# zju3dv/clean-pvnet

Hardware: NVIDIA H100
Metric: ransac_vote_throughput (higher is better)
Workload: dtype f32

## Files before the change

clean_pvnet_b200/csrc/api.cu:

```cuda
#include <cmath>
#include <cstdarg>
#include <cstdio>
#include <cstring>
#include <new>
#include <vector>
#include "kernels.h"

using namespace pvb;

namespace {

thread_local char g_err[512] = "";

int fail(int code, const char *fmt, ...)
{
    va_list ap;
    va_start(ap, fmt);
    vsnprintf(g_err, sizeof(g_err), fmt, ap);
    va_end(ap);
    return code;
}

int cuda_fail(cudaError_t e, const char *what)
{
// ... 12 lines not shown
thread_local std::vector<cudaEvent_t> g_prof_pool;

cudaEvent_t prof_event()
{
    if (!g_prof_pool.empty()) { cudaEvent_t e = g_prof_pool.back(); g_prof_pool.pop_back(); return e; }
    cudaEvent_t e = nullptr;
    cudaEventCreate(&e);
    return e;
}

ProfCall *prof_begin(bool head)
{
    if (g_prof_every <= 0 || (g_prof_tick++ % (unsigned)g_prof_every) != 0) return nullptr;
    ProfCall pc;
    for (auto &e : pc.ev) e = prof_event();
    pc.head = head;
    g_prof_calls.push_back(pc);
    return &g_prof_calls.back();
}

inline void prof_start(ProfCall *pc, int stage, cudaStream_t st) { if (pc && stage == 0) cudaEventRecord(pc->ev[0], st); }
inline void prof_end(ProfCall *pc, int stage, cudaStream_t st) { if (pc) cudaEventRecord(pc->ev[stage + 1], st); }

int default_capacity(const pvb_desc *d)
{
    const long long HW = (long long)d->H * d->W;
    long long cap = d->capacity;
    if (cap <= 0) {
        const long long mn = d->max_num < 0 ? 0 : d->max_num;
        cap = mn + (long long)ceil(8.0 * sqrt((double)mn)) + 64;
    }
    if (cap > HW) cap = HW;
    cap = (cap + 31) / 32 * 32;
    return (int)cap;
}

int check_desc(const pvb_desc *d)
{
    if (!d) return fail(PVB_ERR_INVALID, "descriptor is NULL");
    if (d->B < 0 || d->H <= 0 || d->W <= 0 || d->K <= 0 || d->hn <= 0)
        return fail(PVB_ERR_INVALID, "bad shape B=%d H=%d W=%d K=%d hn=%d", d->B, d->H, d->W, d->K, d->hn);
    if ((long long)d->H * d->W > (1ll << 30)) return fail(PVB_ERR_INVALID, "image too large (H*W > 2^30)");
    if (d->B > 65535 || d->K > 65535) return fail(PVB_ERR_INVALID, "B and K must be <= 65535");
    if ((long long)d->K * ((d->hn + 511) / 512) > 65535) return fail(PVB_ERR_INVALID, "K*ceil(hn/512) must be <= 65535");
    if (d->mask_dtype < PVB_MASK_U8 || d->mask_dtype > PVB_MASK_F64) return fail(PVB_ERR_INVALID, "bad mask_dtype %d", d->mask_dtype);
    if (d->select_mode != PVB_SELECT_BYTE && d->select_mode != PVB_SELECT_EQ1)
        return fail(PVB_ERR_INVALID, "bad select_mode %d", d->select_mode);
    return PVB_OK;
}

int make_layout(const pvb_desc *d, pvb_layout *L)
{
    const int rc = check_desc(d);
    if (rc) return rc;
    const size_t B = (size_t)d->B, K = (size_t)d->K, hn = (size_t)d->hn;
    const int nwords = (int)(((long long)d->H * d->W + 31) / 32);
    const int nblocks = (nwords + 127) / 128;
    const int cap = default_capacity(d);
    const int splits = refit_splits_for(cap);
    size_t off = 0;
    auto take = [&](size_t bytes) { const size_t o = off; off = align_up(off + bytes); return o; };
    L->status = take(4 * sizeof(int));
    L->fgsum = take(B * sizeof(unsigned long long));
    L->nz = take(B * sizeof(int));
    L->tn = take(B * sizeof(int));
    L->state = take(B * sizeof(int));
    L->refit_ticket = take(B * K * sizeof(int));
    L->ticket = take(B * sizeof(int));
    L->blocktot = take(B * nblocks * sizeof(int));
    L->bits = take(B * nwords * sizeof(uint32_t));
    L->xy = take(B * cap * sizeof(float2));
    L->dirs = take(B * K * cap * sizeof(float2));
    L->hyp = take(B * K * hn * sizeof(float2));
    L->counts = take(B * K * hn * sizeof(int));
    L->win = take(B * K * sizeof(float2));
    L->refit_partial = take(B * K * splits * 5 * sizeof(double));
    const size_t ncells = (size_t)((d->H + PRUNE_CELL - 1) / PRUNE_CELL) * ((d->W + PRUNE_CELL - 1) / PRUNE_CELL);
    L->prune_cells = take(B * K * ncells * PRUNE_REC * sizeof(int));
    L->prune_key = take(B * K * hn * sizeof(int));
    L->prune_list = take(2 * B * K * hn * sizeof(int));
    L->prune_len = take(2 * B * K * sizeof(int));
    take(B * K * ncells * 4 * PRUNE_REC * sizeof(int));
    take(B * K * hn * sizeof(int));
    L->total = off;
    L->nwords = nwords;
    L->nblocks = nblocks;
    L->capacity = cap;
    L->refit_splits = splits;
    L->prune_ncells = (int)ncells;
    return PVB_OK;
}

struct Plan {
    pvb_layout L;
    SelectArgs s;
    VoteArgs v;
    float2 *win;
    RefitScratch refit;
    PruneArgs prune;
};

int make_plan(const pvb_desc *d, const void *mask, const float *vertex, const int32_t *idxs,
              const float *selection, void *ws, size_t ws_bytes, uint32_t tag_idx, uint32_t tag_sel, Plan *P)
{
    int rc = make_layout(d, &P->L);
    if (rc) return rc;
    if (!mask || !vertex) return fail(PVB_ERR_INVALID, "mask/vertex is NULL");
    if (!ws || ws_bytes < P->L.total) return fail(PVB_ERR_WORKSPACE, "workspace too small: need %zu bytes, got %zu", P->L.total, ws_bytes);
    if (reinterpret_cast<uintptr_t>(ws) & 255u) return fail(PVB_ERR_WORKSPACE, "workspace must be 256-byte aligned");
    char *w = static_cast<char *>(ws);
    const pvb_layout &L = P->L;
    SelectArgs &s = P->s;
    s.mask = mask; s.mask_dtype = d->mask_dtype; s.select_mode = d->select_mode;
    s.msb = d->mask_stride[0]; s.msy = d->mask_stride[1]; s.msx = d->mask_stride[2];
    s.vertex = vertex;
    for (int i = 0; i < 5; ++i) s.vs[i] = d->vertex_stride[i];
    s.selection = selection;
    s.B = d->B; s.H = d->H; s.W = d->W; s.K = d->K; s.nwords = L.nwords; s.nblocks = L.nblocks; s.cap = L.capacity;
    s.min_num = d->min_num; s.max_num = d->max_num; s.img_base = d->img_base;
    s.seed = d->seed; s.tag_sel = d->rng_tag_sel ? (uint32_t)d->rng_tag_sel : tag_sel;
    s.rowwise_gather = 0;
    s.seg_classes = 0; s.seg_cs = 0; s.mask_out = nullptr;
    s.bits = reinterpret_cast<uint32_t *>(w + L.bits);
    s.blocktot = reinterpret_cast<unsigned *>(w + L.blocktot);
    s.ticket = reinterpret_cast<int *>(w + L.ticket);
    s.fgsum = reinterpret_cast<unsigned long long *>(w + L.fgsum);
    s.nz = reinterpret_cast<int *>(w + L.nz);
    s.tn = reinterpret_cast<int *>(w + L.tn);
    s.state = reinterpret_cast<int *>(w + L.state);
    s.status = reinterpret_cast<int *>(w + L.status);
    s.xy = reinterpret_cast<float2 *>(w + L.xy);
    s.dirs = reinterpret_cast<float2 *>(w + L.dirs);
    VoteArgs &v = P->v;
    v.B = d->B; v.K = d->K; v.hn = d->hn; v.cap = L.capacity; v.W = d->W; v.H = d->H;
    v.thresh = d->inlier_thresh;
    v.tn = s.tn; v.state = s.state; v.xy = s.xy;
    v.dirs = s.dirs; v.idxs = idxs; v.seed = d->seed;
    v.tag_idx = d->rng_tag_idx ? (uint32_t)d->rng_tag_idx : tag_idx;
    v.img_base = d->img_base;
    v.hyp = reinterpret_cast<float2 *>(w + L.hyp);
    v.counts = reinterpret_cast<int *>(w + L.counts);
    P->win = reinterpret_cast<float2 *>(w + L.win);
    P->refit.partial = reinterpret_cast<double *>(w + L.refit_partial);
    P->refit.ticket = reinterpret_cast<int *>(w + L.refit_ticket);
    P->refit.splits = L.refit_splits;
    P->prune.cells = reinterpret_cast<int *>(w + L.prune_cells);
    P->prune.key = reinterpret_cast<int *>(w + L.prune_key);
    P->prune.list = reinterpret_cast<int *>(w + L.prune_list);
    P->prune.len = reinterpret_cast<int *>(w + L.prune_len);
    const size_t BK = (size_t)d->B * d->K;
    const size_t prune_sub = align_up(L.prune_len + 2 * BK * sizeof(int));
    P->prune.sub = reinterpret_cast<int *>(w + prune_sub);
    P->prune.b2 = reinterpret_cast<int *>(w + align_up(prune_sub + BK * L.prune_ncells * 4 * PRUNE_REC * sizeof(int)));
    P->prune.ticket = P->refit.ticket;
    P->prune.ncx = (d->W + PRUNE_CELL - 1) / PRUNE_CELL;
    P->prune.ncells = L.prune_ncells;
    P->prune.cos_w = P->prune.sin_w = 0.f;
    return PVB_OK;
}

cudaError_t run_vote(const Plan &P, bool prune, cudaStream_t st)
{
    PruneArgs q = P.prune;
    if (prune && prune_setup(P.v, q)) return launch_vote_pruned(P.v, q, st);
    return launch_vote(P.v, false, false, st);
}

int run_select(const Plan &P, cudaStream_t st)
{
    cudaError_t e = cudaMemsetAsync(P.s.status, 0, P.L.bits, st);
    if (e != cudaSuccess) return cuda_fail(e, "memset(header)");
    e = launch_select(P.s, st);
    if (e != cudaSuccess) return cuda_fail(e, "select kernels");
    return PVB_OK;
}

int run_front(const Plan &P, bool prune, cudaStream_t st, ProfCall *pc)
{
    prof_start(pc, PVB_STAGE_SELECT, st);
    int rc = run_select(P, st);
    if (rc) return rc;
    prof_end(pc, PVB_STAGE_SELECT, st);
    prof_start(pc, PVB_STAGE_GENERATE, st);
    cudaError_t e = launch_generate(P.v, true, st);
    if (e != cudaSuccess) return cuda_fail(e, "generate kernel");
    prof_end(pc, PVB_STAGE_GENERATE, st);
    prof_start(pc, PVB_STAGE_VOTE, st);
    e = run_vote(P, prune, st);
    if (e != cudaSuccess) return cuda_fail(e, "vote kernel");
    prof_end(pc, PVB_STAGE_VOTE, st);
    return PVB_OK;
}

}

struct pvb_exchange {
    int rank, world, slots, device;
    size_t bytes_per_rank;
    size_t status_off, total;
    char *local;
    char *peer[PVB_MAX_PEERS];
    bool ipc_opened[PVB_MAX_PEERS];
    bool connected;
};

namespace {

int exchange_push_args(pvb_exchange *ex, uint64_t seq, size_t nbytes, PeerPush *pp)
{
    memset(pp, 0, sizeof(*pp));
    if (!ex) return PVB_OK;
    if (!ex->connected) return fail(PVB_ERR_INVALID, "exchange is not connected (pvb_exchange_connect*)");
    if (seq == 0 || (uint32_t)seq == 0) return fail(PVB_ERR_INVALID, "seq must be >= 1 and not a multiple of 2^32");
    if (nbytes > ex->bytes_per_rank) return fail(PVB_ERR_INVALID, "result block (%zu bytes) exceeds the exchange's bytes_per_rank (%zu)", nbytes, ex->bytes_per_rank);
    const size_t slot = (size_t)((seq - 1) % (uint64_t)ex->slots);
    const size_t words = ex->bytes_per_rank / sizeof(float);
    pp->world = ex->world;
    pp->seq = (uint32_t)seq;
    for (int r = 0; r < ex->world; ++r)
        pp->recv[r] = reinterpret_cast<uint2 *>(ex->peer[r]) + (slot * ex->world + ex->rank) * words;
    return PVB_OK;
}

size_t mask_elt_bytes(int dt)
{
    switch (dt) {
    case PVB_MASK_U8: case PVB_MASK_I8: return 1;
    case PVB_MASK_I16: return 2;
    case PVB_MASK_I32: case PVB_MASK_F32: return 4;
    default: return 8;
    }
}

}

extern "C" {
// ... 918 lines not shown
```

clean_pvnet_b200/csrc/kernels.h:

```cpp
#pragma once
#include <cuda_runtime.h>
#include <stdint.h>
#include "../../include/pvnet_vote_b200.h"
#include "pnp_core.cuh"

namespace pvb {

struct SelectArgs {
    const void *mask;
    int mask_dtype, select_mode;
    long long msb, msy, msx;
    const float *vertex;
    long long vs[5];
    const float *selection;
    int B, H, W, K, nwords, nblocks, cap, min_num, max_num, img_base;
    int rowwise_gather;
    int seg_classes;
    long long seg_cs;
    long long *mask_out;
    uint64_t seed;
    uint32_t tag_sel;
    uint32_t *bits;
    unsigned *blocktot;
    int *ticket;
    unsigned long long *fgsum;
    int *nz, *tn, *state, *status;
    float2 *xy, *dirs;
};
cudaError_t launch_select(const SelectArgs &a, cudaStream_t st);

struct VoteArgs {
    int B, K, hn, cap, W, H;
    float thresh;
    const int *tn;
    const int *state;
    const float2 *xy;
    const float2 *dirs;
    const int32_t *idxs;
    uint64_t seed;
    uint32_t tag_idx;
    int img_base;
    float2 *hyp;
    int *counts;
};
cudaError_t launch_generate(const VoteArgs &a, bool chained, cudaStream_t st);
cudaError_t launch_vote(const VoteArgs &a, bool zero_counts, bool chained, cudaStream_t st);

constexpr int PRUNE_CELL = 32;
constexpr int PRUNE_SUB = PRUNE_CELL / 2;
constexpr int PRUNE_NBIN = 128;
constexpr int PRUNE_REC = 4 + PRUNE_NBIN / 2;
constexpr int PRUNE_M = 128;
constexpr int PRUNE_MAX_HN = 2048;
constexpr int PRUNE_MIN_UNITS = 32;
static_assert(PRUNE_CELL * PRUNE_CELL < 65536, "a cell's prefix counts fit 16 bits");
struct PruneArgs {
    int *cells;
    int *sub;
    int *key;
    int *b2;
    int *list;
    int *len;
    int *ticket;
    int ncx, ncells;
    float cos_w, sin_w;
};
bool prune_setup(const VoteArgs &a, PruneArgs &q);
cudaError_t launch_vote_pruned(const VoteArgs &a, const PruneArgs &q, cudaStream_t st);
cudaError_t launch_vote_list(const VoteArgs &a, const int *list, const int *len, int max_len, cudaStream_t st);
cudaError_t launch_vote_list_slices(const VoteArgs &a, const int *list, const int *len, int max_len, cudaStream_t st);
void set_vote_tuning(int variant);
void set_gather_tuning(int mode);
struct RefitScratch { double *partial; int *ticket; int splits; };
int refit_splits_for(int cap);
constexpr int PVB_MAX_PEERS = 16;
struct PeerPush {
    int world;
    unsigned int seq;
    uint2 *recv[PVB_MAX_PEERS];
};
cudaError_t launch_refit(const VoteArgs &a, float2 *win, const RefitScratch &rs, float *out_kpt, const PeerPush &pp,
                         cudaStream_t st);
struct ExchangeCounts { int n[PVB_MAX_PEERS]; };
cudaError_t launch_exchange_wait(const uint2 *recv, unsigned int seq, float *out, int world, int stride_words,
                                 const ExchangeCounts &counts, unsigned long long timeout_ns, int *status, cudaStream_t st);
cudaError_t launch_covariance(const VoteArgs &a, const float *mean, float *out_cov, const PeerPush &pp, cudaStream_t st);

cudaError_t launch_pnp_weights(const float *cov, float *w, int n, cudaStream_t st);

constexpr int PNP_FUSED_MAX_PN = 64;
struct PnpArgs {
    const double *pts2d;
    const double *wgt2d;
    const float *kpt2d;
    const float *cov;
    const float *weights;
    float *weights_out;
    const double *pts3d;
    const double *K;
    const double *init_rt;
    double *init_out;
    double *result_rt;
    int *info;
    double *pose;
    int n, pn;
    long long pts3d_stride, k_stride;
    PnpOptions opt;
};
cudaError_t launch_pnp_batch(const PnpArgs &a, cudaStream_t st);
cudaError_t launch_pnp_iterative(const PnpArgs &a, cudaStream_t st);

struct NnPlan { int qchunks, nsplit, slice; };
NnPlan nn_plan(int b, int pn1, int pn2);
size_t nn_workspace_bytes(int b, int pn1, int pn2);
size_t add_metric_workspace_bytes(int n, int pn, int syn, size_t *partial_offset);
cudaError_t launch_nearest_point(const float *ref, const float *que, int *idxs, int b, int pn1, int pn2, int dim,
                                 bool exclude_self, void *workspace, cudaStream_t st);
cudaError_t launch_add_metric(const double *model, const double *pose_pred, const double *pose_gt, double *mean_dist, int n,
                              int pn, bool syn, void *workspace, cudaStream_t st);
size_t pose_metrics_workspace_bytes(int n, int pn);
cudaError_t launch_pose_metrics(const double *model, const double *pose_pred, const double *pose_gt, const double *K,
                                long long k_stride, double *proj2d, double *trans_cm, double *angle_deg, int n, int pn,
                                void *workspace, cudaStream_t st);
cudaError_t launch_mask_iou(const void *pred, int pred_dtype, const long long *ps, const void *gt, int gt_dtype,
                            const long long *gs, long long *inter, long long *uni, int B, int H, int W, cudaStream_t st);

size_t render_workspace_bytes(int n, int F);
cudaError_t launch_render_depth(const float *pts, int V, const int *faces, int F, const double *poses, int n,
                                const double *K, long long k_stride, float *depth, int H, int W, double znear,
                                double zfar, void *workspace, cudaStream_t st);
struct VsdArgs {
    const float *depth_test, *depth_est, *depth_gt;
    const int *pairs;
    const double *K;
    long long k_stride;
    int n, B, n_est, n_gt, est_base, gt_base, H, W;
    double delta, tau;
    double *e;
};
size_t vsd_workspace_bytes(int n);
cudaError_t launch_vsd(const VsdArgs &a, void *workspace, cudaStream_t st);

struct VoteLossArgs {
    const float *pred;
    long long ps[4];
    const void *mask;
    int mask_dtype;
    long long msb, msy, msx;
    const double *kpt;
    int B, H, W, K;
    float *out;
    double *partial;
    long long *wpart;
// ... 19 lines not shown
```

clean_pvnet_b200/csrc/prune.cu:

```cuda
#include <cmath>
#include <math_constants.h>
#include "common.cuh"
#include "kernels.h"

namespace pvb {

template <bool EXACT = false>
__device__ __forceinline__ float pseudo_angle(float x, float y)
{
    const bool xn = x < 0.f, yn = y < 0.f;
    const float num = (xn == yn) ? fabsf(y) : fabsf(x), den = fabsf(x) + fabsf(y);
    const float off = yn ? (xn ? 2.f : 3.f) : (xn ? 1.f : 0.f);
    return off + (EXACT ? __fdiv_rn(num, den) : __fdividef(num, den));
}

__device__ int first_row_at(const float2 *xy, int n, float y)
{
    const int lane = threadIdx.x & 31;
    int lo = 0, hi = n;
    while (hi > lo) {
        const int step = (hi - lo + 31) / 32;
        const int p = lo + lane * step;
        const unsigned below = __ballot_sync(0xffffffffu, p < hi && __ldg(&xy[p].y) < y);
        const int nb = __popc(below);
// ... 214 lines not shown
            __syncthreads();
        }
    }
}

__device__ void plan_pass1(const VoteArgs &a, const PruneArgs &q, size_t bk, int *s_key, int *s_cnt, int *s_w, int *s_sel)
{
    const int tid = threadIdx.x, lane = tid & 31, warp = tid >> 5;
    const int hn = a.hn, M = min(PRUNE_M, hn);
    int *key = q.key + bk * hn;
    int top = 0;
    for (int h = tid; h < hn; h += BOUND_THREADS) {
        const int v = __ldcg(key + h);
        s_key[h] = v;
        top = max(top, v);
    }
    top = __reduce_max_sync(0xffffffffu, top);
    if (lane == 0) s_w[warp] = top;
    __syncthreads();
    for (int w = 0; w < BOUND_WARPS; ++w) top = max(top, s_w[w]);
    int thr = 0, need = M;
    for (int hi = 32 - __clz(top | 1); hi > 0;) {
        const int lo = max(0, hi - 8);
        for (int i = tid; i < 256; i += BOUND_THREADS) s_cnt[i] = 0;
        __syncthreads();
        for (int h = tid; h < hn; h += BOUND_THREADS) {
            const int v = s_key[h];
            if ((v >> hi) == (thr >> hi)) atomicAdd(&s_cnt[(v >> lo) & ((1 << (hi - lo)) - 1)], 1);
        }
        __syncthreads();
        if (warp == 0) {
            int c[8], own = 0;
#pragma unroll
            for (int e = 0; e < 8; ++e) { c[e] = s_cnt[8 * lane + e]; own += c[e]; }
            int suf = own;
#pragma unroll
            for (int o = 1; o < 32; o <<= 1) {
                const int t = __shfl_down_sync(0xffffffffu, suf, o);
                if (lane + o < 32) suf += t;
            }
            const unsigned ok = __ballot_sync(0xffffffffu, suf >= need);
            if (lane == 31 - __clz(ok)) {
                int above = suf - own;
#pragma unroll
                for (int e = 7; e >= 0; --e) {
                    if (above + c[e] >= need) { s_sel[0] = 8 * lane + e; s_sel[1] = need - above; break; }
                    above += c[e];
                }
            }
        }
        __syncthreads();
        thr |= s_sel[0] << lo;
        need = s_sel[1];
        hi = lo;
    }
    const int per = (hn + 32 * BOUND_WARPS - 1) / (32 * BOUND_WARPS) * 32;
    const int h0 = warp * per, h1 = min(hn, h0 + per);
    int gt = 0, eq = 0;
    for (int h = h0 + lane; h - lane < h1; h += 32) {
        const int v = h < h1 ? s_key[h] : -1;
        gt += __popc(__ballot_sync(0xffffffffu, v > thr));
        eq += __popc(__ballot_sync(0xffffffffu, v == thr));
    }
    int *s_gt = s_w, *s_eq = s_w + BOUND_WARPS;
    __syncthreads();
    if (lane == 0) { s_gt[warp] = gt; s_eq[warp] = eq; }
    __syncthreads();
    gt = eq = 0;
    for (int w = 0; w < warp; ++w) { gt += s_gt[w]; eq += s_eq[w]; }
    int *list = q.list + bk * hn;
    const unsigned below = (1u << lane) - 1u;
    for (int h = h0 + lane; h - lane < h1; h += 32) {
        const int v = h < h1 ? s_key[h] : -1;
        const unsigned mg = __ballot_sync(0xffffffffu, v > thr), me = __ballot_sync(0xffffffffu, v == thr);
        const int g = gt + __popc(mg & below), e = eq + __popc(me & below);
        if (v > thr || (v == thr && e < need)) {
            list[g + min(e, need)] = h;
            key[h] = -1;
        }
        gt += __popc(mg);
        eq += __popc(me);
    }
    if (tid == 0) q.len[bk] = M;
}

__global__ void __launch_bounds__(BOUND_THREADS, 2048 / BOUND_THREADS)
prune_bound_kernel(VoteArgs a, PruneArgs q)
{
    const int tid = threadIdx.x;
    const int part = tid / BOUND_HYPS, hl = tid % BOUND_HYPS;
    const int h = blockIdx.x * BOUND_HYPS + hl, k = blockIdx.y, b = blockIdx.z;
    const size_t bk = (size_t)b * a.K + k;
    const int tn = max(0, min(a.tn[b], a.cap));
    __shared__ __align__(16) int s_rec[2][STAGE_RECS * PRUNE_REC];
    __shared__ int s_idx[3 * BOUND_THREADS];
    __shared__ int s_part[BOUND_SPLIT][BOUND_HYPS];
    __shared__ int s_w[2 * BOUND_WARPS];
    __shared__ int s_sel[2];
    const float2 hp = (h < a.hn) ? a.hyp[bk * a.hn + h] : make_float2(0.f, 0.f);
    grid_dep_wait();
    grid_dep_launch_dependents();
    int bound = 0;
    stream_records<BOUND_THREADS>(q.cells + bk * q.ncells * PRUNE_REC, PRUNE_REC, q.ncells, &s_rec[0][0], s_idx, s_w,
                                  [&](const int *rec, int n) {
        const int r0 = part * n / BOUND_SPLIT, r1 = (part + 1) * n / BOUND_SPLIT;
        count_bound(q, rec + r0 * PRUNE_REC, r1 - r0, hp.x, hp.y, bound);
    });
    if (part > 0) s_part[part][hl] = bound;
    __syncthreads();
    if (part == 0 && h < a.hn) {
#pragma unroll
        for (int p = 1; p < BOUND_SPLIT; ++p) bound += s_part[p][hl];
        q.key[bk * a.hn + h] = bounded(hp) ? bound : tn;
        q.b2[bk * a.hn + h] = 0;
    }
    __threadfence();
    __syncthreads();
    if (tid == 0) {
        s_sel[0] = (atomicAdd(q.ticket + bk, 1) == (int)gridDim.x - 1);
        if (s_sel[0]) q.ticket[bk] = 0;
    }
    __syncthreads();
    if (!s_sel[0]) return;
    __threadfence();
    plan_pass1(a, q, bk, &s_rec[0][0], &s_rec[0][0] + PRUNE_MAX_HN, s_w, s_sel);
}

constexpr int NEXT_THREADS = 256;
constexpr int NEXT_CTAS = 8;
constexpr int NEXT_CAND_BYTES = sizeof(float2) + sizeof(int) + sizeof(unsigned short);
static_assert(PRUNE_MAX_HN <= 65536, "candidate indices fit 16 bits");

__device__ __forceinline__ int cta_scan(bool flag, int *s_warp, int *total)
{
    const int lane = threadIdx.x & 31, warp = threadIdx.x >> 5;
    const unsigned m = __ballot_sync(0xffffffffu, flag);
    __syncthreads();
    if (lane == 0) s_warp[warp] = __popc(m);
    __syncthreads();
    int before = 0, tot = 0;
    for (int w = 0; w < NEXT_THREADS / 32; ++w) {
        const int c = s_warp[w];
        before += (w < warp) ? c : 0;
        tot += c;
    }
    *total = tot;
    return before + __popc(m & ((1u << lane) - 1u));
}

__global__ void __launch_bounds__(NEXT_THREADS)
prune_next_kernel(VoteArgs a, PruneArgs q)
{
    const int x = blockIdx.x, k = blockIdx.y, b = blockIdx.z, tid = threadIdx.x;
    const size_t bk = (size_t)b * a.K + k;
    const size_t BK = (size_t)a.B * a.K;
    const int hn = a.hn;
    __shared__ __align__(16) int s_rec[2 * STAGE_RECS * PRUNE_REC];
    __shared__ int s_idx[3 * NEXT_THREADS];
    __shared__ int s_warp[NEXT_THREADS / 32];
    __shared__ int s_last;
    extern __shared__ __align__(16) unsigned char s_dyn[];
    const int ncap = hn - PRUNE_M;
    float2 *s_hyp = reinterpret_cast<float2 *>(s_dyn);
    int *s_b2 = reinterpret_cast<int *>(s_hyp + ncap);
    unsigned short *s_cand = reinterpret_cast<unsigned short *>(s_b2 + ncap);
    const int *key = q.key + bk * hn;
    const float2 *hyp = a.hyp + bk * hn;
    int *b2 = q.b2 + bk * hn;
    static_assert(PRUNE_M <= NEXT_THREADS, "one pass-1 entry per thread");
    int L = 0;
    {
        const int *counts = a.counts + bk * hn;
        int best = 0;
        const int n1 = q.len[bk];
        const int h1 = tid < n1 ? q.list[bk * hn + tid] : -1;
        grid_dep_wait();
        grid_dep_launch_dependents();
        if (h1 >= 0) best = __ldcg(counts + h1);
        best = __reduce_max_sync(0xffffffffu, best);
        if ((tid & 31) == 0) s_warp[tid >> 5] = best;
        __syncthreads();
        for (int w = 0; w < NEXT_THREADS / 32; ++w) L = max(L, s_warp[w]);
    }
    int nc = 0;
    for (int h0 = 0; h0 < hn && L > 0; h0 += NEXT_THREADS) {
        const int h = h0 + tid;
        const float2 hp = h < hn ? hyp[h] : make_float2(0.f, 0.f);
        const bool f = h < hn && key[h] >= L && bounded(hp);
        int n;
        const int pos = nc + cta_scan(f, s_warp, &n);
        if (f) { s_cand[pos] = (unsigned short)h; s_hyp[pos] = hp; s_b2[pos] = 0; }
        nc += n;
    }
    if (nc > 0) {
        __syncthreads();
        const int P = max(1, NEXT_THREADS / nc);
        const int *sub = q.sub + (bk * q.ncells * 4 + x) * PRUNE_REC;
        const int nsub = (4 * q.ncells - x + NEXT_CTAS - 1) / NEXT_CTAS;
        stream_records<NEXT_THREADS>(sub, NEXT_CTAS * PRUNE_REC, nsub, s_rec, s_idx, s_warp, [&](const int *rec, int n) {
            for (int it = tid; it < nc * P; it += NEXT_THREADS) {
                const int j = it % nc, p = it / nc;
                const int r0 = p * n / P, r1 = (p + 1) * n / P;
                if (r1 == r0) continue;
                const float2 hp = s_hyp[j];
                int bound = 0;
                count_bound(q, rec + r0 * PRUNE_REC, r1 - r0, hp.x, hp.y, bound);
                if (bound) atomicAdd(&s_b2[j], bound);
            }
        });
        for (int j = tid; j < nc; j += NEXT_THREADS)
            if (s_b2[j]) atomicAdd(&b2[s_cand[j]], s_b2[j]);
    }
    __threadfence();
    __syncthreads();
    if (tid == 0) {
        s_last = (atomicAdd(q.ticket + bk, 1) == (int)gridDim.x - 1);
        if (s_last) q.ticket[bk] = 0;
    }
    __syncthreads();
    if (!s_last) return;
    __threadfence();
    int *list = q.list + (BK + bk) * hn;
    int base = 0;
    for (int h0 = 0; h0 < hn; h0 += NEXT_THREADS) {
        const int h = h0 + tid;
        const bool f = h < hn && key[h] >= L && (L == 0 || !bounded(hyp[h]) || __ldcg(b2 + h) >= L);
        int n;
        const int pos = base + cta_scan(f, s_warp, &n);
        if (f) list[pos] = h;
        base += n;
    }
    if (tid == 0) q.len[BK + bk] = base;
}

bool prune_setup(const VoteArgs &a, PruneArgs &q)
{
    const double t = (double)a.thresh;
    if (!(t > 0.0 && t < 1.0) || a.hn <= PRUNE_M || a.hn > PRUNE_MAX_HN) return false;
    if ((long long)a.B * a.K < PRUNE_MIN_UNITS) return false;
    if ((long long)a.K * ((a.hn + 63) / 64) > 65535) return false;
    const double u = ldexp(1.0, -24);
    const double w = acos(fmax(-1.0, t - 64.0 * u)) + 1e-5;
    if (!(w < 1.5)) return false;
    q.cos_w = nextafterf((float)cos(w), 0.f);
    q.sin_w = nextafterf((float)sin(w), 1.f);
    return true;
}

cudaError_t launch_vote_pruned(const VoteArgs &a, const PruneArgs &q, cudaStream_t st)
{
    const size_t BK = (size_t)a.B * a.K;
    const int nbands = (a.H + PRUNE_CELL - 1) / PRUNE_CELL;
    cudaError_t e = launch_chained(true, prune_hist_kernel, dim3(nbands, a.K, a.B), HIST_THREADS, 0, st, a, q);
    if (e == cudaSuccess)
        e = launch_chained(true, prune_bound_kernel, dim3((a.hn + BOUND_HYPS - 1) / BOUND_HYPS, a.K, a.B), BOUND_THREADS, 0, st,
                           a, q);
    if (e == cudaSuccess) e = launch_vote_list_slices(a, q.list, q.len, PRUNE_M, st);
    if (e == cudaSuccess)
        e = launch_chained(true, prune_next_kernel, dim3(NEXT_CTAS, a.K, a.B), NEXT_THREADS,
                           (size_t)(a.hn - PRUNE_M) * NEXT_CAND_BYTES, st, a, q);
    if (e != cudaSuccess) return e;
    return launch_vote_list(a, q.list + BK * a.hn, q.len + BK, a.hn - PRUNE_M, st);
}

}
```

clean_pvnet_b200/csrc/vote.cu:

```cuda
#include <atomic>
#include <math_constants.h>
#include "common.cuh"
#include "kernels.h"

namespace pvb {

__global__ void __launch_bounds__(256)
generate_kernel(VoteArgs a)
{
    grid_dep_wait();
    grid_dep_launch_dependents();
    const int h = blockIdx.x * 256 + threadIdx.x;
    if (h >= a.hn) return;
    const int k = blockIdx.y, b = blockIdx.z;
    const int tn = min(a.tn[b], a.cap);
    float x = 0.f, y = 0.f;
    if (tn > 0) {
        int t0, t1;
        if (a.idxs) {
            const int2 t = __ldg(reinterpret_cast<const int2 *>(a.idxs) + ((size_t)b * a.hn + h) * a.K + k);
            t0 = t.x; t1 = t.y;
        } else {
            const uint4 r = philox4x32_10(make_uint4((uint32_t)h, (uint32_t)k, (uint32_t)(a.img_base + b), a.tag_idx),
                                          make_uint2((uint32_t)a.seed, (uint32_t)(a.seed >> 32)));
// ... 321 lines not shown
    const int t0 = blockIdx.x * LIST_TILE;
    const size_t bk = (size_t)b * a.K + k;
    const int nh = __ldcg(len + bk);
    if (t0 >= tn || nh <= 0) return;
    const int n = min(LIST_TILE, tn - t0);
    const int tid = threadIdx.x, lane = tid & 31, warp = tid >> 5;
    const int *lst = list + bk * a.hn;
    const float2 *hyp = a.hyp + bk * a.hn;
    const float2 *xy = a.xy + (size_t)b * a.cap + t0;
    const float2 *dk = a.dirs + bk * a.cap + t0;

    int h = 0;
    float2 hq = make_float2(0.f, 0.f);
    if (tid < nh) { h = __ldcg(lst + tid); hq = hyp[h]; }
    float4 ra[LIST_PPT];
    float2 rb[LIST_PPT];
    float ox, oy, cmax;
    {
        float2 v[LIST_PPT], c[LIST_PPT];
        load_tile<LIST_NT, LIST_PPT>(dk, xy, n, v, c, s_box, ox, oy, cmax);
#pragma unroll
        for (int r = 0; r < LIST_PPT; ++r) {
            cone_record(tid + r * LIST_NT < n, v[r], c[r], ox, oy, cmax, cone.kappa, ra[r], rb[r]);
            s_a[tid + r * LIST_NT] = ra[r]; s_b[tid + r * LIST_NT] = rb[r];
        }
    }
    unsigned *tally = s_tally[warp];
    for (int c0 = 0; c0 < nh; c0 += LIST_CHUNK) {
        const int ns = min(LIST_CHUNK, nh - c0);
        if (c0 > 0 && tid < ns) { h = __ldcg(lst + c0 + tid); hq = hyp[h]; }
        if (tid < ns) {
            const float3 f = hyp_frame(hq, ox, oy, cmax, cone);
            s_h[tid] = make_float4(f.x, f.y, f.z, __int_as_float(h));
        } else {
            s_h[tid] = make_float4(0.f, 0.f, 0.f, 0.f);
        }
        __syncthreads();
        for (int s = 0; s < ns; s += LIST_U) {
            float4 q[LIST_U];
            int neg[LIST_U];
            float mn[LIST_U];
            bool flag = false;
#pragma unroll
            for (int u = 0; u < LIST_U; ++u) {
                q[u] = s_h[s + u];
                neg[u] = 0;
                mn[u] = CUDART_INF_F;
#pragma unroll
                for (int r = 0; r < LIST_PPT; ++r) {
                    const float m = cone_margin(ra[r], rb[r], q[u].x, q[u].y);
                    neg[u] += (int)(__float_as_uint(m) >> 31);
                    mn[u] = fminf(mn[u], fabsf(m));
                }
                flag |= mn[u] < q[u].z;
            }
            if (flag) {
#pragma unroll
                for (int u = 0; u < LIST_U; ++u)
                    if (mn[u] < q[u].z) neg[u] += list_exact(q[u], s_a, s_b, hyp, dk, xy, n, cone.thresh);
            }
#pragma unroll
            for (int u = 0; u < LIST_U; u += 2) {
                const unsigned t = __reduce_add_sync(0xffffffffu, (unsigned)(LIST_PPT - neg[u]) | ((unsigned)(LIST_PPT - neg[u + 1]) << 16));
                if (lane == 0) tally[(s + u) / 2] = t;
            }
        }
        __syncthreads();
        if (tid < ns) {
            int cnt = 0;
#pragma unroll
            for (int w = 0; w < NW; ++w) cnt += (int)((s_tally[w][tid / 2] >> (16 * (tid & 1))) & 0xffffu);
            if (cnt) atomicAdd(a.counts + bk * a.hn + __float_as_int(s_h[tid].w), cnt);
        }
    }
}

cudaError_t launch_vote_list(const VoteArgs &a, const int *list, const int *len, int max_len, cudaStream_t st)
{
    if (max_len <= 0) return cudaSuccess;
    dim3 g((a.cap + LIST_TILE - 1) / LIST_TILE, a.K, a.B);
    return launch_chained(true, vote_list_kernel, g, LIST_NT, 0, st, a, make_cone(a.thresh), list, len);
}

cudaError_t launch_vote_list_slices(const VoteArgs &a, const int *list, const int *len, int max_len, cudaStream_t st)
{
    constexpr int HPT = 4, NT = 128, TILE = 1024;
    static_assert(HPT * 32 == PRUNE_M, "pass 1 is one slice");
    if (max_len <= 0) return cudaSuccess;
    VoteK p;
    p.a = a;
    p.cone = make_cone(a.thresh);
    p.list = list;
    p.len = len;
    const int slices = (max_len + HPT * 32 - 1) / (HPT * 32);
    dim3 g((a.cap + TILE - 1) / TILE, a.K * slices, a.B);
    return launch_chained(true, vote_kernel<HPT, NT, 8, TILE, 1>, g, NT, 0, st, p);
}

template <int NV>
__device__ __forceinline__ void peer_push(const PeerPush &pp, size_t bk, const float (&v)[NV])
{
    for (int r = 0; r < pp.world; ++r) {
        uint2 *dst = pp.recv[r] + bk * NV;
#pragma unroll
        for (int i = 0; i < NV; ++i)
            asm volatile("st.volatile.global.v2.u32 [%0], {%1, %2};" ::"l"(dst + i), "r"(__float_as_uint(v[i])), "r"(pp.seq) : "memory");
    }
}

constexpr int RF_THREADS = 128;
constexpr int RF_CHUNK = 2048;

int refit_splits_for(int cap) { return (cap + RF_CHUNK - 1) / RF_CHUNK; }

__device__ __forceinline__ bool vote_winner(float vx, float vy, float cx, float cy, float hx, float hy,
                                            const ConeParams &cone)
{
    const float dx = __fsub_rn(hx, cx), dy = __fsub_rn(hy, cy);
    const float n1sq = fmaf(vx, vx, vy * vy);
    const float S = fabsf(dx) + fabsf(dy);
    const float m = cone.kappa * fmaf(vx, dx, vy * dy) - fabsf(fmaf(vx, dy, -(vy * dx)));
    const float thr = cone.band * S;
    const bool safe = (n1sq > 1e-10f) && (n1sq < 1e8f) && (S >= 2e-6f) && (S <= 1e6f) &&
                      (m * m > thr * thr * n1sq * 1.0001f);
    return safe ? (m > 0.f) : vote_exact(vx, vy, cx, cy, hx, hy, cone.thresh);
}

__global__ void __launch_bounds__(RF_THREADS)
refit_kernel(VoteArgs a, float2 *__restrict__ win, RefitScratch rs, float *__restrict__ out, ConeParams cone, PeerPush pp)
{
    grid_dep_wait();
    const int split = blockIdx.x, k = blockIdx.y, b = blockIdx.z;
    const int tid = threadIdx.x, lane = tid & 31, warp = tid >> 5;
    constexpr int NW = RF_THREADS / 32;
    const int tn = min(a.tn[b], a.cap);
    const size_t bk = (size_t)b * a.K + k;
    __shared__ int s_c[NW], s_h[NW];
    __shared__ double s_acc[NW][5];
    __shared__ int s_last;
    float2 res = make_float2(0.f, 0.f);
    if (a.state[b] != 0 || tn <= 0) {
        if (split != 0) return;
        if (tid == 0) { out[bk * 2] = 0.f; out[bk * 2 + 1] = 0.f; win[bk] = make_float2(0.f, 0.f); }
    } else {
        const int nsplit = (tn + RF_CHUNK - 1) / RF_CHUNK;
        if (split >= nsplit) return;
        const int *counts = a.counts + bk * a.hn;
        int bc = -1, bh = 0x7fffffff;
        for (int h = tid; h < a.hn; h += RF_THREADS) {
            const int c = counts[h];
            if (c > bc) { bc = c; bh = h; }
        }
#pragma unroll
        for (int o = 16; o > 0; o >>= 1) {
            const int oc = __shfl_xor_sync(0xffffffffu, bc, o), oh = __shfl_xor_sync(0xffffffffu, bh, o);
            if (oc > bc || (oc == bc && oh < bh)) { bc = oc; bh = oh; }
        }
        if (lane == 0) { s_c[warp] = bc; s_h[warp] = bh; }
        __syncthreads();
#pragma unroll
        for (int w = 0; w < NW; ++w)
            if (s_c[w] > bc || (s_c[w] == bc && s_h[w] < bh)) { bc = s_c[w]; bh = s_h[w]; }
        const float2 wpt = (bc > 0) ? a.hyp[bk * a.hn + bh] : make_float2(0.f, 0.f);
        if (split == 0 && tid == 0) win[bk] = wpt;

        const float2 *xy = a.xy + (size_t)b * a.cap;
        const float2 *dk = a.dirs + bk * a.cap;
        const int t_end = min(tn, (split + 1) * RF_CHUNK);
        double a00 = 0, a01 = 0, a11 = 0, b0 = 0, b1 = 0;
        constexpr int RU = 4;
        for (int t0 = split * RF_CHUNK + tid; t0 < t_end; t0 += RF_THREADS * RU) {
            float2 v[RU], c[RU];
#pragma unroll
            for (int u = 0; u < RU; ++u) {
                const int t = t0 + u * RF_THREADS;
                v[u] = make_float2(0.f, 0.f); c[u] = make_float2(0.f, 0.f);
                if (t < t_end) { v[u] = __ldg(dk + t); c[u] = __ldg(xy + t); }
            }
#pragma unroll
// ... 112 lines not shown
```

Baseline: 294,900.

## Vote first-pass hypotheses in spatial groups with box-based sure/unsure pixel culling

After pass-1 planning, the 128 first-pass hypotheses are recursively split by median along their bounding box's longer axis into four spatially coherent groups of 32, and each group's bounding box is written to a new workspace table. A new group vote kernel tests every pixel in a tile against the cone at the group box corners. Pixels that are surely inliers for the whole group are counted in bulk, and only undecided pixels are compacted into a list and tested per hypothesis, with an exact fallback near the margin. This replaces the sliced vote kernel to skip most per-pixel per-hypothesis work, at the cost of extra planning, synchronisation and more complex code that must match the exact counts.

```diff
diff --git a/clean_pvnet_b200/csrc/api.cu b/clean_pvnet_b200/csrc/api.cu
--- a/clean_pvnet_b200/csrc/api.cu
+++ b/clean_pvnet_b200/csrc/api.cu
@@ -118,6 +118,7 @@
     L->prune_len = take(2 * B * K * sizeof(int));
     take(B * K * ncells * 4 * PRUNE_REC * sizeof(int));
     take(B * K * hn * sizeof(int));
+    take(B * K * PRUNE_GROUP_WORDS * sizeof(int));
     L->total = off;
     L->nwords = nwords;
     L->nblocks = nblocks;
@@ -187,7 +188,9 @@
     const size_t BK = (size_t)d->B * d->K;
     const size_t prune_sub = align_up(L.prune_len + 2 * BK * sizeof(int));
     P->prune.sub = reinterpret_cast<int *>(w + prune_sub);
-    P->prune.b2 = reinterpret_cast<int *>(w + align_up(prune_sub + BK * L.prune_ncells * 4 * PRUNE_REC * sizeof(int)));
+    const size_t prune_b2 = align_up(prune_sub + BK * L.prune_ncells * 4 * PRUNE_REC * sizeof(int));
+    P->prune.b2 = reinterpret_cast<int *>(w + prune_b2);
+    P->prune.group = reinterpret_cast<int *>(w + align_up(prune_b2 + BK * d->hn * sizeof(int)));
     P->prune.ticket = P->refit.ticket;
     P->prune.ncx = (d->W + PRUNE_CELL - 1) / PRUNE_CELL;
     P->prune.ncells = L.prune_ncells;
diff --git a/clean_pvnet_b200/csrc/kernels.h b/clean_pvnet_b200/csrc/kernels.h
--- a/clean_pvnet_b200/csrc/kernels.h
+++ b/clean_pvnet_b200/csrc/kernels.h
@@ -54,6 +54,10 @@
 constexpr int PRUNE_MAX_HN = 2048;
 constexpr int PRUNE_MIN_UNITS = 32;
 static_assert(PRUNE_CELL * PRUNE_CELL < 65536, "a cell's prefix counts fit 16 bits");
+constexpr int PRUNE_GROUP = 32;
+constexpr int PRUNE_NGROUP = PRUNE_M / PRUNE_GROUP;
+constexpr int PRUNE_GROUP_WORDS = PRUNE_M + 4 * PRUNE_NGROUP;
+static_assert(PRUNE_M % PRUNE_GROUP == 0 && (PRUNE_M / PRUNE_GROUP & (PRUNE_M / PRUNE_GROUP - 1)) == 0, "groups halve");
 struct PruneArgs {
     int *cells;
     int *sub;
@@ -61,6 +65,7 @@
     int *b2;
     int *list;
     int *len;
+    int *group;
     int *ticket;
     int ncx, ncells;
     float cos_w, sin_w;
@@ -68,7 +73,7 @@
 bool prune_setup(const VoteArgs &a, PruneArgs &q);
 cudaError_t launch_vote_pruned(const VoteArgs &a, const PruneArgs &q, cudaStream_t st);
 cudaError_t launch_vote_list(const VoteArgs &a, const int *list, const int *len, int max_len, cudaStream_t st);
-cudaError_t launch_vote_list_slices(const VoteArgs &a, const int *list, const int *len, int max_len, cudaStream_t st);
+cudaError_t launch_vote_groups(const VoteArgs &a, const int *group, cudaStream_t st);
 void set_vote_tuning(int variant);
 void set_gather_tuning(int mode);
 struct RefitScratch { double *partial; int *ticket; int splits; };
diff --git a/clean_pvnet_b200/csrc/prune.cu b/clean_pvnet_b200/csrc/prune.cu
--- a/clean_pvnet_b200/csrc/prune.cu
+++ b/clean_pvnet_b200/csrc/prune.cu
@@ -320,6 +320,82 @@
         eq += __popc(me);
     }
     if (tid == 0) q.len[bk] = M;
+}
+
+__device__ void plan_groups(const VoteArgs &a, const PruneArgs &q, int *s)
+{
+    static_assert(PRUNE_M <= BOUND_THREADS && PRUNE_M % 32 == 0 && PRUNE_GROUP % 32 == 0, "groups are whole warps");
+    constexpr int MW = PRUNE_M / 32;
+    const int tid = threadIdx.x, lane = tid & 31, warp = tid >> 5;
+    const size_t bk = (size_t)blockIdx.z * a.K + blockIdx.y;
+    int2 *s_key = reinterpret_cast<int2 *>(s);
+    float *s_x = reinterpret_cast<float *>(s + 2 * PRUNE_M), *s_y = s_x + PRUNE_M;
+    int *s_h = s + 4 * PRUNE_M, *s_p = s + 5 * PRUNE_M;
+    float (*s_wb)[4] = reinterpret_cast<float (*)[4]>(s + 6 * PRUNE_M);
+    __syncthreads();
+    float x = 0.f, y = 0.f;
+    int h = 0, p = tid;
+    bool ok = false;
+    if (tid < PRUNE_M) {
+        h = __ldcg(q.list + bk * a.hn + tid);
+        const float2 hp = a.hyp[bk * a.hn + h];
+        x = hp.x; y = hp.y;
+        ok = bounded(hp);
+    }
+    auto warp_box = [&](float &x0, float &x1, float &y0, float &y1) {
+        x0 = ok ? x : CUDART_INF_F; x1 = ok ? x : -CUDART_INF_F; y0 = ok ? y : CUDART_INF_F; y1 = ok ? y : -CUDART_INF_F;
+#pragma unroll
+        for (int o = 16; o > 0; o >>= 1) {
+            x0 = fminf(x0, __shfl_xor_sync(0xffffffffu, x0, o)); x1 = fmaxf(x1, __shfl_xor_sync(0xffffffffu, x1, o));
+            y0 = fminf(y0, __shfl_xor_sync(0xffffffffu, y0, o)); y1 = fmaxf(y1, __shfl_xor_sync(0xffffffffu, y1, o));
+        }
+    };
+    for (int n = PRUNE_M; n > PRUNE_GROUP; n >>= 1) {
+        float x0 = 0.f, x1 = 0.f, y0 = 0.f, y1 = 0.f;
+        if (warp < MW) {
+            warp_box(x0, x1, y0, y1);
+            if (lane == 0) { s_wb[warp][0] = x0; s_wb[warp][1] = x1; s_wb[warp][2] = y0; s_wb[warp][3] = y1; }
+        }
+        __syncthreads();
+        float c = 0.f;
+        const int g0 = tid / n * n;
+        if (tid < PRUNE_M) {
+            for (int w = g0 / 32; w < (g0 + n) / 32; ++w) {
+                x0 = fminf(x0, s_wb[w][0]); x1 = fmaxf(x1, s_wb[w][1]); y0 = fminf(y0, s_wb[w][2]); y1 = fmaxf(y1, s_wb[w][3]);
+            }
+            c = ok ? (x1 - x0 >= y1 - y0 ? x : y) : CUDART_INF_F;
+            s_key[tid] = make_int2(__float_as_int(c), p);
+        }
+        __syncthreads();
+        if (tid < PRUNE_M) {
+            int r = g0;
+#pragma unroll 8
+            for (int j = g0; j < g0 + n; ++j) {
+                const int2 kj = s_key[j];
+                const float cj = __int_as_float(kj.x);
+                r += cj < c || (cj == c && kj.y < p);
+            }
+            s_x[r] = x; s_y[r] = y; s_h[r] = h; s_p[r] = p | (ok ? 0 : 1 << 30);
+        }
+        __syncthreads();
+        if (tid < PRUNE_M) {
+            x = s_x[tid]; y = s_y[tid]; h = s_h[tid];
+            p = s_p[tid] & ((1 << 30) - 1); ok = s_p[tid] < (1 << 30);
+        }
+        __syncthreads();
+    }
+    int *tab = q.group + bk * PRUNE_GROUP_WORDS;
+    if (warp < MW) {
+        tab[tid] = h;
+        float x0, x1, y0, y1;
+        warp_box(x0, x1, y0, y1);
+        if (__any_sync(0xffffffffu, !ok)) x0 = x1 = y0 = y1 = CUDART_NAN_F;
+        if (lane == 0) {
+            static_assert(PRUNE_GROUP == 32, "one group per warp");
+            reinterpret_cast<int4 *>(tab + PRUNE_M)[warp] =
+                make_int4(__float_as_int(x0), __float_as_int(x1), __float_as_int(y0), __float_as_int(y1));
+        }
+    }
 }
 
 __global__ void __launch_bounds__(BOUND_THREADS, 2048 / BOUND_THREADS)
@@ -362,6 +438,7 @@
     if (!s_sel[0]) return;
     __threadfence();
     plan_pass1(a, q, bk, &s_rec[0][0], &s_rec[0][0] + PRUNE_MAX_HN, s_w, s_sel);
+    plan_groups(a, q, &s_rec[0][0]);
 }
 
 constexpr int NEXT_THREADS = 256;
@@ -493,7 +570,7 @@
     if (e == cudaSuccess)
         e = launch_chained(true, prune_bound_kernel, dim3((a.hn + BOUND_HYPS - 1) / BOUND_HYPS, a.K, a.B), BOUND_THREADS, 0, st,
                            a, q);
-    if (e == cudaSuccess) e = launch_vote_list_slices(a, q.list, q.len, PRUNE_M, st);
+    if (e == cudaSuccess) e = launch_vote_groups(a, q.group, st);
     if (e == cudaSuccess)
         e = launch_chained(true, prune_next_kernel, dim3(NEXT_CTAS, a.K, a.B), NEXT_THREADS,
                            (size_t)(a.hn - PRUNE_M) * NEXT_CAND_BYTES, st, a, q);
diff --git a/clean_pvnet_b200/csrc/vote.cu b/clean_pvnet_b200/csrc/vote.cu
--- a/clean_pvnet_b200/csrc/vote.cu
+++ b/clean_pvnet_b200/csrc/vote.cu
@@ -427,19 +427,179 @@
     return launch_chained(true, vote_list_kernel, g, LIST_NT, 0, st, a, make_cone(a.thresh), list, len);
 }
 
-cudaError_t launch_vote_list_slices(const VoteArgs &a, const int *list, const int *len, int max_len, cudaStream_t st)
-{
-    constexpr int HPT = 4, NT = 128, TILE = 1024;
-    static_assert(HPT * 32 == PRUNE_M, "pass 1 is one slice");
-    if (max_len <= 0) return cudaSuccess;
-    VoteK p;
-    p.a = a;
-    p.cone = make_cone(a.thresh);
-    p.list = list;
-    p.len = len;
-    const int slices = (max_len + HPT * 32 - 1) / (HPT * 32);
-    dim3 g((a.cap + TILE - 1) / TILE, a.K * slices, a.B);
-    return launch_chained(true, vote_kernel<HPT, NT, 8, TILE, 1>, g, NT, 0, st, p);
+constexpr int GV_NT = 128;
+constexpr int GV_TILE = 1024;
+constexpr int GV_PPT = GV_TILE / GV_NT;
+constexpr int GV_HPT = 4;
+constexpr int GV_LANES = PRUNE_GROUP / GV_HPT;
+constexpr int GV_TEAMS = GV_NT / GV_LANES;
+static_assert(PRUNE_GROUP % GV_HPT == 0 && 32 % GV_LANES == 0, "a warp holds whole teams");
+static_assert(GV_TILE <= 65535, "pixel indices fit 16 bits");
+
+__global__ void __launch_bounds__(GV_NT, 8)
+group_vote_kernel(const VoteArgs a, const ConeParams cone, const int *__restrict__ group)
+{
+    __shared__ __align__(16) float4 s_a[GV_TILE + 1];
+    __shared__ __align__(16) float2 s_b[GV_TILE + 1];
+    __shared__ __align__(4) unsigned short s_list[GV_TILE];
+    __shared__ int s_nu[2], s_in[2], s_votes[2][PRUNE_GROUP];
+    __shared__ float2 s_q[PRUNE_M];
+    __shared__ float4 s_gbox[PRUNE_NGROUP];
+    __shared__ float s_box[4][GV_NT / 32];
+    const int b = blockIdx.z, k = blockIdx.y;
+    const int tn = min(a.tn[b], a.cap);
+    const int t0 = blockIdx.x * GV_TILE;
+    const size_t bk = (size_t)b * a.K + k;
+    if (t0 >= tn) { grid_dep_wait(); return; }
+    const int n = min(GV_TILE, tn - t0);
+    const int tid = threadIdx.x, lane = tid & 31;
+    const float2 *hyp = a.hyp + bk * a.hn;
+    const float2 *xy = a.xy + (size_t)b * a.cap + t0;
+    const float2 *dk = a.dirs + bk * a.cap + t0;
+
+    float ox, oy, cmax;
+    {
+        float2 v[GV_PPT], c[GV_PPT];
+        load_tile<GV_NT, GV_PPT>(dk, xy, n, v, c, s_box, ox, oy, cmax);
+#pragma unroll
+        for (int r = 0; r < GV_PPT; ++r) {
+            const int i = tid + r * GV_NT;
+            if (i < n) {
+                float4 ra;
+                float2 rb;
+                cone_record(true, v[r], c[r], ox, oy, cmax, cone.kappa, ra, rb);
+                s_a[i] = ra; s_b[i] = rb;
+            }
+        }
+    }
+    if (tid == 0) { s_a[GV_TILE] = make_float4(0.f, 0.f, -1e30f, 0.f); s_b[GV_TILE] = make_float2(0.f, 0.f); }
+    if (tid < 2) { s_nu[tid] = 0; s_in[tid] = 0; }
+    if (tid < 2 * PRUNE_GROUP) (&s_votes[0][0])[tid] = 0;
+
+    grid_dep_wait();
+    grid_dep_launch_dependents();
+    const int *members = group + bk * PRUNE_GROUP_WORDS;
+    const int team = tid / GV_LANES, tl = tid % GV_LANES;
+    const unsigned below = (1u << lane) - 1u;
+    static_assert(PRUNE_M <= GV_NT, "one table entry per thread");
+    if (tid < PRUNE_M) s_q[tid] = hyp[__ldcg(members + tid)];
+    if (tid < PRUNE_NGROUP) {
+        const int4 bx = __ldcg(reinterpret_cast<const int4 *>(members + PRUNE_M) + tid);
+        s_gbox[tid] = make_float4(__int_as_float(bx.x), __int_as_float(bx.y), __int_as_float(bx.z), __int_as_float(bx.w));
+    }
+    __syncthreads();
+
+    for (int g = 0; g < PRUNE_NGROUP; ++g) {
+        const int pb = g & 1;
+        const int *mem = members + g * PRUNE_GROUP;
+        const float2 *gq = s_q + g * PRUNE_GROUP;
+        const int hid = tid < PRUNE_GROUP ? __ldcg(mem + tid) : 0;
+        float hxc[GV_HPT], hyc[GV_HPT], dl[GV_HPT];
+#pragma unroll
+        for (int j = 0; j < GV_HPT; ++j) {
+            const float3 f = hyp_frame(gq[tl + j * GV_LANES], ox, oy, cmax, cone);
+            hxc[j] = f.x; hyc[j] = f.y; dl[j] = f.z;
+        }
+        const float4 bx = s_gbox[g];
+        const float x0 = bx.x, x1 = bx.y, y0 = bx.z, y1 = bx.w;
+        const float3 cr[4] = {hyp_frame(make_float2(x0, y0), ox, oy, cmax, cone), hyp_frame(make_float2(x1, y0), ox, oy, cmax, cone),
+                              hyp_frame(make_float2(x0, y1), ox, oy, cmax, cone), hyp_frame(make_float2(x1, y1), ox, oy, cmax, cone)};
+        const float d = fmaxf(fmaxf(cr[0].z, cr[1].z), fmaxf(cr[2].z, cr[3].z));
+        int sure = 0;
+        unsigned und = 0;
+#pragma unroll
+        for (int r = 0; r < GV_PPT; ++r) {
+            const int i = tid + r * GV_NT;
+            if (i < n) {
+                const float4 ra = s_a[i];
+                const float2 rb = s_b[i];
+                float mn = CUDART_INF_F, fp = -CUDART_INF_F, fm = -CUDART_INF_F;
+#pragma unroll
+                for (int q = 0; q < 4; ++q) {
+                    const float ap = fmaf(ra.x, cr[q].x, fmaf(ra.y, cr[q].y, ra.z));
+                    const float pp = fmaf(ra.w, cr[q].x, fmaf(rb.x, cr[q].y, rb.y));
+                    mn = fminf(mn, ap - fabsf(pp));
+                    fp = fmaxf(fp, ap + pp);
+                    fm = fmaxf(fm, ap - pp);
+                }
+                const bool in = mn >= d;
+                sure += in;
+                und |= (unsigned)(!in && !(fp <= -d) && !(fm <= -d)) << r;
+            }
+        }
+        unsigned bal[GV_PPT];
+        int nw = 0;
+#pragma unroll
+        for (int r = 0; r < GV_PPT; ++r) { bal[r] = __ballot_sync(0xffffffffu, (und >> r) & 1u); nw += __popc(bal[r]); }
+        int base = 0;
+        if (lane == 0 && nw) base = atomicAdd(&s_nu[pb], nw);
+        base = __shfl_sync(0xffffffffu, base, 0);
+#pragma unroll
+        for (int r = 0; r < GV_PPT; ++r) {
+            if ((und >> r) & 1u) s_list[base + __popc(bal[r] & below)] = (unsigned short)(tid + r * GV_NT);
+            base += __popc(bal[r]);
+        }
+        sure = __reduce_add_sync(0xffffffffu, sure);
+        if (lane == 0 && sure) atomicAdd(&s_in[pb], sure);
+        __syncthreads();
+
+        const int nu = s_nu[pb];
+        if (tid < 2) { s_nu[pb ^ 1] = 0; s_in[pb ^ 1] = 0; }
+        if (tid < PRUNE_GROUP) s_votes[pb ^ 1][tid] = 0;
+        int votes[GV_HPT];
+        float mn[GV_HPT];
+#pragma unroll
+        for (int j = 0; j < GV_HPT; ++j) { votes[j] = 0; mn[j] = CUDART_INF_F; }
+        int mine = 0;
+        const unsigned *s_pairs = reinterpret_cast<const unsigned *>(s_list);
+        unsigned pr = 2 * team < nu ? s_pairs[team] : 0u;
+        for (int e = 2 * team; e < nu; e += 2 * GV_TEAMS) {
+            const int i0 = pr & 0xffffu, i1 = e + 1 < nu ? (int)(pr >> 16) : GV_TILE;
+            pr = e + 2 * GV_TEAMS < nu ? s_pairs[(e >> 1) + GV_TEAMS] : 0u;
+            const float4 ra0 = s_a[i0], ra1 = s_a[i1];
+            const float2 rb0 = s_b[i0], rb1 = s_b[i1];
+            mine += 2;
+#pragma unroll
+            for (int j = 0; j < GV_HPT; ++j) {
+                const float m0 = cone_margin(ra0, rb0, hxc[j], hyc[j]);
+                const float m1 = cone_margin(ra1, rb1, hxc[j], hyc[j]);
+                votes[j] -= (int)(__float_as_uint(m0) >> 31);
+                votes[j] -= (int)(__float_as_uint(m1) >> 31);
+                mn[j] = fminf(mn[j], fminf(fabsf(m0), fabsf(m1)));
+            }
+        }
+#pragma unroll
+        for (int j = 0; j < GV_HPT; ++j) {
+            votes[j] += mine;
+            if (mn[j] < dl[j]) {
+                const float2 q = gq[tl + j * GV_LANES];
+                for (int e = 2 * team; e < nu; ++e) {
+                    const int i = s_list[e];
+                    const float m = cone_margin(s_a[i], s_b[i], hxc[j], hyc[j]);
+                    if (fabsf(m) < dl[j]) {
+                        const float2 vv = __ldg(dk + i), cc = __ldg(xy + i);
+                        votes[j] += (vote_exact(vv.x, vv.y, cc.x, cc.y, q.x, q.y, cone.thresh) ? 1 : 0) -
+                                    (1 - (int)(__float_as_uint(m) >> 31));
+                    }
+                    if (e & 1) e += 2 * GV_TEAMS - 2;
+                }
+            }
+#pragma unroll
+            for (int o = GV_LANES; o < 32; o <<= 1) votes[j] += __shfl_xor_sync(0xffffffffu, votes[j], o);
+            if (lane < GV_LANES) atomicAdd(&s_votes[pb][tl + j * GV_LANES], votes[j]);
+        }
+        __syncthreads();
+        if (tid < PRUNE_GROUP) {
+            const int cnt = s_in[pb] + s_votes[pb][tid];
+            if (cnt) atomicAdd(a.counts + bk * a.hn + hid, cnt);
+        }
+    }
+}
+
+cudaError_t launch_vote_groups(const VoteArgs &a, const int *group, cudaStream_t st)
+{
+    dim3 g((a.cap + GV_TILE - 1) / GV_TILE, a.K, a.B);
+    return launch_chained(true, group_vote_kernel, g, GV_NT, 0, st, a, make_cone(a.thresh), group);
 }
 
 template <int NV>
```

After: 298,500, median of 6. 1.01x the previous value.
